# LPD-EPFL-ML/X-MAP

Hardware: AMD Instinct MI355X
Metric: item_sim_pairs_per_s (higher is better)
Workload: dtype f64

## Files before the change

### x-map_amd/csrc/tilesort.h

```cpp
#pragma once
#include "common.h"

namespace xmap {
namespace ts {

constexpr int BT = 256;
template <int RW> struct Chunk { static constexpr int CH = RW == 2 ? 4096 : 2048; static constexpr int EPT = CH / BT; };
constexpr int NB_LOG = 7;
constexpr int NB = 1 << NB_LOG;
constexpr int NA_MAX = 256;
constexpr int CAP = 3072;
constexpr int CT = 512;
constexpr int NK_MAX = 520;
constexpr int SL = 2048;
constexpr int LT = 256;

struct Geo {
    int K;
    long long M;
    int KW, ts_log, T, NA;
    int ch;
    const long long *ptr;
    int *tile_key0;
    long long *tile_pos0;
    int *tile_large;
    unsigned long long *curA;
    unsigned long long *curB;
    unsigned *counters;
    int2 *clist;
    int2 *slist;
    long long clist_cap, slist_cap;
};

__device__ __forceinline__ long long measure(const Geo &G, int k, long long p) { return p + (long long)k * G.KW; }

__device__ __forceinline__ void block_scan_2(const unsigned *cnt, unsigned *off, int n, unsigned *wsum) {
    const int tid = threadIdx.x, lane = tid & 63, w = tid >> 6;
    const unsigned a = (2 * tid < n) ? cnt[2 * tid] : 0u, b = (2 * tid + 1 < n) ? cnt[2 * tid + 1] : 0u;
    unsigned inc = a + b;
#pragma unroll
    for (int d = 1; d < 64; d <<= 1) { const unsigned o = __shfl_up(inc, d, 64); if (lane >= d) inc += o; }
    if (lane == 63) wsum[w] = inc;
    __syncthreads();
    unsigned base = 0;
    for (int x = 0; x < w; x++) base += wsum[x];
    const unsigned ex = base + inc - (a + b);
    if (2 * tid < n) off[2 * tid] = ex;
    if (2 * tid + 1 < n) off[2 * tid + 1] = ex + a;
    if (tid == BT - 1) off[n] = base + inc;
    __syncthreads();
}

template <int RW>
struct RecLoader {
    const unsigned long long *__restrict__ in;
    __device__ __forceinline__ bool chunk(long long n_in, long long &i0, long long &i1) const {
        i0 = (long long)blockIdx.x * Chunk<RW>::CH;
        i1 = min(n_in, i0 + Chunk<RW>::CH);
        return true;
    }
    __device__ __forceinline__ void load(long long idx, unsigned long long (&w)[RW]) const {
#pragma unroll
        for (int x = 0; x < RW; x++) w[x] = in[idx * RW + x];
    }
    __device__ __forceinline__ bool keep(const unsigned long long (&)[RW]) const { return true; }
    __device__ __forceinline__ void extra(long long, const unsigned long long (&)[Chunk<RW>::EPT][RW], const bool (&)[Chunk<RW>::EPT]) const {}
};

template <int RW, bool LEVEL_B, typename Loader>
__global__ __launch_bounds__(BT) void k_ts_bin(Geo G, Loader L, long long n_in, unsigned long long *__restrict__ out) {
    constexpr int CH = Chunk<RW>::CH, EPT = Chunk<RW>::EPT;
    constexpr int NBK = LEVEL_B ? 2 * NB : NA_MAX;
    __shared__ unsigned hist[NBK];
    __shared__ unsigned off[NBK + 1];
    __shared__ long long gbase[NBK];
    __shared__ unsigned wsum[BT / 64];
    __shared__ __attribute__((aligned(16))) unsigned long long stage[CH * RW];
    __shared__ unsigned short sbk[CH];
    constexpr int NKB = LEVEL_B ? NB : NA_MAX;
    __shared__ int bkey0[NKB], blarge[LEVEL_B ? NB : 1];
    const int tid = threadIdx.x;
    long long i0, i1;
    int a = 0;
    if (LEVEL_B) {
        if (blockIdx.x >= G.counters[0]) return;
        const int2 c = G.clist[blockIdx.x];
        a = c.x;
        const int t0 = a << NB_LOG, t1 = min(G.T, (a + 1) << NB_LOG);
        i0 = G.tile_pos0[t0] + (long long)c.y * CH;
        i1 = min(G.tile_pos0[t1], i0 + CH);
    } else {
        if (!L.chunk(n_in, i0, i1)) return;
    }
    const int nbk = LEVEL_B ? 2 * NB : G.NA;
    for (int b = tid; b < nbk; b += BT) hist[b] = 0u;
    if (LEVEL_B) {
        for (int b = tid; b < NB; b += BT) { bkey0[b] = G.tile_key0[(a << NB_LOG) + b]; blarge[b] = G.tile_large[(a << NB_LOG) + b]; }
    } else {
        for (int b = tid; b < NA_MAX; b += BT) bkey0[b] = b < G.NA ? G.tile_key0[b << NB_LOG] : 0x7fffffff;
    }
    __syncthreads();
    unsigned long long w[EPT][RW];
    bool on[EPT], rt[EPT];
    unsigned br[EPT];
#pragma unroll
    for (int r = 0; r < EPT; r++) {
        const long long idx = i0 + r * BT + tid;
        on[r] = idx < i1;
        if (on[r]) L.load(idx, w[r]);
        else {
#pragma unroll
            for (int x = 0; x < RW; x++) w[r][x] = 0ull;
        }
        rt[r] = on[r] && L.keep(w[r]);
    }
#pragma unroll
    for (int r = 0; r < EPT; r++) br[r] = 0u;
#pragma unroll
    for (int d = NKB / 2; d > 0; d >>= 1)
#pragma unroll
        for (int r = 0; r < EPT; r++)
            if (bkey0[br[r] + d] <= (int)(unsigned)w[r][0]) br[r] += d;
    if (LEVEL_B) {
#pragma unroll
        for (int r = 0; r < EPT; r++)
            if (blarge[br[r]] == (int)(unsigned)w[r][0]) br[r] |= NB;
    }
#pragma unroll
    for (int r = 0; r < EPT; r++)
        if (rt[r]) br[r] = (br[r] << 16) | atomicAdd(&hist[br[r]], 1u);
    __syncthreads();
    block_scan_2(hist, off, nbk, wsum);
    for (int b = tid; b < nbk; b += BT) {
        const unsigned c = hist[b];
        if (!c) continue;
        long long start;
        unsigned long long *cur;
        if (LEVEL_B) {
            const int t = (a << NB_LOG) | (b & (NB - 1));
            if (b >= NB) { start = G.ptr[G.tile_large[t]]; cur = &G.curB[(size_t)G.T + t]; }
            else { start = G.tile_pos0[t]; cur = &G.curB[t]; }
        } else {
            start = G.tile_pos0[b << NB_LOG];
            cur = &G.curA[b];
        }
        gbase[b] = (start + (long long)atomicAdd(cur, (unsigned long long)c) - (long long)off[b]) * RW;
    }
#pragma unroll
    for (int r = 0; r < EPT; r++) {
        if (!rt[r]) continue;
        const unsigned b = br[r] >> 16, s = off[b] + (br[r] & 0xffffu);
#pragma unroll
        for (int x = 0; x < RW; x++) stage[s * RW + x] = w[r][x];
        sbk[s] = (unsigned short)b;
    }
    L.extra(i0, w, on);
    __syncthreads();
    constexpr int VW = RW % 2 == 0 ? 2 : 1;
    const int nw = (int)off[nbk] * RW;
#pragma unroll 4
    for (int q = tid * VW; q < nw; q += BT * VW) {
        unsigned long long *o = out + (gbase[sbk[q / RW]] + q);
#pragma unroll
        for (int x = 0; x < VW; x++) o[x] = stage[q + x];
    }
}

struct TileHead { int k0, nk, large; long long pos0; int n; };
__device__ __forceinline__ TileHead tile_head(const Geo &G, int t) {
    TileHead h;
    h.k0 = G.tile_key0[t];
    const int k1 = G.tile_key0[t + 1];
    h.large = G.tile_large[t];
    const int ks1 = h.large >= 0 ? h.large : k1;
    h.nk = ks1 - h.k0;
    h.pos0 = G.tile_pos0[t];
    const long long pos1 = h.large >= 0 ? G.ptr[h.large] : G.tile_pos0[t + 1];
    h.n = (int)(pos1 - h.pos0);
    return h;
}

}
}
```

### x-map_amd/csrc/tri.h

```cpp
#pragma once
#include "common.h"
#include "tilesort.h"

namespace xmap {

constexpr int T_SLOTS = 1024;
constexpr int HMAX = 1024;
constexpr int SMALL_BOUND = 96;
constexpr int MID_BOUND = 384;

constexpr int N_CLASSES = 5;
constexpr int WIDE_MIN = 2048;
__host__ __device__ __forceinline__ int class_rank(int cls) {
    return cls == 4 ? 0 : (cls == 0 ? 1 : (cls == 2 ? 2 : (cls == 3 ? 3 : 4)));
}

__device__ __forceinline__ double weighted(double cs, int n, int cap) {
    const int mn = n < cap ? n : cap;
    return 1.0 * cs * (double)mn / (double)cap;
}
__device__ __forceinline__ unsigned long long ls_key(double d) {
    return (d != d) ? 0x7ff8000000000000ull : (unsigned long long)__double_as_longlong(d);
}

struct RaterRec { int e0; int pos_ge; float rating; int user; };
struct UbWide { int item_ge; int pad; double rating; };
struct RaterRecWide { int e0; int pos_ge; double rating; };

constexpr int COO_SHARDS = 4096;

int mirror_counts(hipStream_t st, int n_items, long long range_cap, int n_ranges, const unsigned long long *cur, const int *coo_i,
                  const int *coo_j, bool skip_self, int *part, int *counts, FillList *fills = nullptr);
void ts_geometry(int K, long long M, int ch, ts::Geo &G);
int ts_prepare(hipStream_t st, ts::Geo &G, const long long *ptr, FillList *fills = nullptr);
extern template __global__ void ts::k_ts_bin<3, true, ts::RecLoader<3>>(ts::Geo, ts::RecLoader<3>, long long, unsigned long long *__restrict__);

}
```

### x-map_amd/csrc/tri_layout.hip

```cpp
#include "tri.h"
#include "item_stats.h"

namespace xmap {

__device__ __forceinline__ unsigned long long wkey(int n, int item) {
    return ((unsigned long long)(unsigned)n << 32) | (unsigned)item;
}

constexpr int HIST_LDS = 2048;
constexpr int HIST_PER = 16;
__global__ __launch_bounds__(256) void k_hist(int I, const long long *iptr, int HB, int *hist) {
    __shared__ int loc[HIST_LDS];
    for (int t = threadIdx.x; t < HIST_LDS; t += 256) loc[t] = 0;
    __syncthreads();
    const long long base = (long long)blockIdx.x * 256 * HIST_PER;
    for (int q = 0; q < HIST_PER; q++) {
        const long long i = base + (long long)q * 256 + threadIdx.x;
        if (i < I) {
            long long n = iptr[i + 1] - iptr[i];
            int bin = n < HB - 1 ? (int)n : HB - 1;
            if (bin < HIST_LDS) atomicAdd(&loc[bin], 1); else atomicAdd(&hist[bin], 1);
        }
    }
    __syncthreads();
// ... 305 lines not shown
        int d = 0;
        if (u < U) { a = uptr[u]; d = (int)(uptr[u + 1] - a); }
        const bool small = d <= 16;
        int wmax = small ? d : 0;
#pragma unroll
        for (int m = 32; m >= 16; m >>= 1) wmax = max(wmax, __shfl_xor(wmax, m, 64));
        wmax = rl32(wmax, 0);
        if (wmax > 0) {
            unsigned long long key = 0ull;
            int px = 0;
            long long py = 0;
            if (small && gl < d) sort_entry3<WIDE>(uitem, ur32, ur64, cnt, a + gl, key, px, py);
            bitonic_desc3<WIDE>(pow2_at_least(wmax), gl, key, px, py);
            if (small && gl < d) emit_entry3<WIDE>(a, d, gl, u, px, py, ub, srec);
        }
    }
    for (int q = 0; q < 4; q++) {
        const long long u = u0 + q;
        if (u >= U) break;
        const long long a = uptr[u];
        const int d = (int)(uptr[u + 1] - a);
        if (d <= 16) continue;
        if (d <= 64) {
            unsigned long long key = 0ull;
            int px = 0;
            long long py = 0;
            if (lane < d) sort_entry3<WIDE>(uitem, ur32, ur64, cnt, a + lane, key, px, py);
            bitonic_desc3<WIDE>(pow2_at_least(d), lane, key, px, py);
            if (lane < d) emit_entry3<WIDE>(a, d, lane, u, px, py, ub, srec);
            continue;
        }
        unsigned long long *keys = d <= SORT_LDS ? lkeys[uniform((int)(threadIdx.x >> 6))] : ub_key + a;
        for (int p = lane; p < d; p += 64) {
            unsigned long long key;
            int px;
            long long py;
            sort_entry3<WIDE>(uitem, ur32, ur64, cnt, a + p, key, px, py);
            keys[p] = key;
        }
        __threadfence_block();
        for (int p = lane; p < d; p += 64) {
            unsigned long long key;
            int px;
            long long py;
            sort_entry3<WIDE>(uitem, ur32, ur64, cnt, a + p, key, px, py);
            int rank = 0;
            for (int o = 0; o < d; o++) rank += (keys[o] > key) || (keys[o] == key && o < p);
            emit_entry3<WIDE>(a, d, rank, u, px, py, ub, srec);
        }
    }
}

template <bool WIDE>
__device__ __forceinline__ ulonglong2 rater_record(const unsigned long long *w, const long long *uptr) {
    const unsigned user = WIDE ? (unsigned)w[2] : (unsigned)(w[1] >> 32);
    const unsigned e0 = (unsigned)uptr[user];
    ulonglong2 o;
    o.x = (unsigned long long)e0 | (w[0] & 0xffffffff00000000ull);
    o.y = w[1];
    return o;
}

template <bool WIDE>
__global__ __launch_bounds__(ts::CT) void k_rc_tiles(ts::Geo G, const unsigned long long *bufB, const long long *uptr,
                                                     ulonglong2 *rc, unsigned long long *Wp) {
    constexpr int RW = WIDE ? 3 : 2;
    __shared__ unsigned cur[ts::NK_MAX], kst[ts::NK_MAX];
    __shared__ unsigned long long wsum[ts::NK_MAX];
    __shared__ ulonglong2 lrec[ts::CAP];
    const ts::TileHead h = ts::tile_head(G, blockIdx.x);
    if (h.nk <= 0) return;
    for (int x = threadIdx.x; x < h.nk; x += ts::CT) {
        cur[x] = 0u; wsum[x] = 0ull;
        kst[x] = (unsigned)(G.ptr[h.k0 + x] - h.pos0);
    }
    __syncthreads();
    const bool in_lds = h.n <= ts::CAP;
    constexpr int UN = 4;
    for (int base = 0; base < h.n; base += ts::CT * UN) {
        unsigned long long w[UN][RW];
        bool on[UN];
#pragma unroll
        for (int t = 0; t < UN; t++) {
            const int idx = base + t * ts::CT + threadIdx.x;
            on[t] = idx < h.n;
            const size_t o = (size_t)(h.pos0 + (on[t] ? idx : 0)) * RW;
#pragma unroll
            for (int x = 0; x < RW; x++) w[t][x] = bufB[o + x];
        }
#pragma unroll
        for (int t = 0; t < UN; t++) {
            if (!on[t]) continue;
            const int kk = (int)((unsigned)w[t][0]) - h.k0;
            const unsigned q = kst[kk] + atomicAdd(&cur[kk], 1u);
            atomicAdd(&wsum[kk], (unsigned long long)((unsigned)(w[t][0] >> 32) & 0x7fffffffu));
            const ulonglong2 o = rater_record<WIDE>(w[t], uptr);
            if (in_lds) lrec[q] = o; else rc[h.pos0 + q] = o;
        }
    }
    __syncthreads();
    if (in_lds)
        for (int q = threadIdx.x; q < h.n; q += ts::CT) rc[h.pos0 + q] = lrec[q];
    for (int x = threadIdx.x; x < h.nk; x += ts::CT) Wp[h.k0 + x] = wsum[x];
}

template <bool WIDE>
__global__ __launch_bounds__(ts::LT) void k_rc_large(ts::Geo G, const unsigned long long *bufB, const long long *uptr,
                                                     ulonglong2 *rc, unsigned long long *Wp) {
    constexpr int RW = WIDE ? 3 : 2;
    if (blockIdx.x >= G.counters[1]) return;
    const int2 sl = G.slist[blockIdx.x];
    const long long lo = G.ptr[sl.x] + (long long)sl.y * ts::SL;
    const long long hi = min(G.ptr[sl.x + 1], lo + ts::SL);
    unsigned long long sum = 0ull;
    for (long long p = lo + threadIdx.x; p < hi; p += ts::LT) {
        unsigned long long w[RW];
#pragma unroll
        for (int x = 0; x < RW; x++) w[x] = bufB[(size_t)p * RW + x];
        sum += (unsigned long long)((unsigned)(w[0] >> 32) & 0x7fffffffu);
        rc[p] = rater_record<WIDE>(w, uptr);
    }
    sum = (unsigned long long)wave_sum_ll((long long)sum);
    if (lane_id() == 0 && sum) atomicAdd(&Wp[sl.x], sum);
}

struct RcSrc {
    RaterRec *rc; const double *u_avg;
    static constexpr bool has_flags = true;
    __device__ __forceinline__ void load(long long p, double &r, int &u) const { const RaterRec x = rc[p]; r = (double)x.rating; u = x.user; }
    __device__ __forceinline__ double uavg(int u) const { return u_avg[u]; }
    __device__ __forceinline__ void set_flag(long long p, bool ge) const { if (ge) rc[p].pos_ge |= (int)0x80000000u; }
};
struct RcWideSrc {
    const RaterRecWide *rc;
    static constexpr bool has_flags = false;
    __device__ __forceinline__ void load(long long p, double &r, int &u) const { r = rc[p].rating; u = 0; }
    __device__ __forceinline__ double uavg(int) const { return 0.0; }
    __device__ __forceinline__ void set_flag(long long, bool) const {}
};

constexpr int STAT_BIG = 512;
constexpr int STAT_CHK = 2048;
struct BigList {
    unsigned *counters;
    int2 *chunks;
    int4 *items;
    double *part;
    long long chunk_cap, item_cap;
};

template <typename Src>
__global__ __launch_bounds__(256) void k_item_stats3(int I, int lo, int hi, const long long *iptr, const Src src, double *info,
                                                     double *norms, BigList B) {
    const int i0 = lo + (blockIdx.x * 4 + uniform((int)(threadIdx.x >> 6))) * 4;
    if (i0 >= hi) return;
    const int lane = lane_id();
    {
        const int i = i0 + (lane >> 4);
        const bool on = i < hi && iptr[i + 1] - iptr[i] <= 64;
        item_stats_group<16, Src, false>(on, i, lane & 15, I, iptr, src, info, norms, nullptr, nullptr);
    }
    for (int t = 0; t < 4; t++) {
        const int i = i0 + t;
        if (i >= hi) break;
        const long long n = iptr[i + 1] - iptr[i];
        if (n <= 64) continue;
        if (n > STAT_BIG) {
            if (lane == 0) {
                const int nch = (int)((n + STAT_CHK - 1) / STAT_CHK);
                const unsigned base = atomicAdd(&B.counters[0], (unsigned)nch);
                const unsigned slot = atomicAdd(&B.counters[1], 1u);
                if ((long long)slot < B.item_cap) B.items[slot] = make_int4(i, (int)base, nch, 0);
                for (int x = 0; x < nch; x++)
                    if ((long long)base + x < B.chunk_cap) B.chunks[base + x] = make_int2(i, x);
            }
            continue;
        }
// ... 112 lines not shown
        FillList F;
        heavy_set_fills(F, n_users, hist, ctl);
        int rc = fill_multi(st, F);
        if (rc) return rc;
    }
    if (I > 0) {
        k_hist<<<dim3((unsigned)((I + 256 * HIST_PER - 1) / (256 * HIST_PER))), dim3(256), 0, st>>>(I, (const long long *)item_ptr, HB, hist);
        XM_LAUNCH_CHECK();
    }
    int rcode = xmap_exclusive_scan_i32_to_i64(stream, hist, pre, HB, nullptr);
    if (rcode) return rcode;
    if (HB - 1 > ch_min) {
        k_threshold<<<dim3((unsigned)((HB + 255) / 256)), dim3(256), 0, st>>>(I, HB, (const long long *)pre, ch_min, ctl);
        XM_LAUNCH_CHECK();
    }
    if (I > 0) {
        k_mark_heavy<<<dim3((unsigned)((I + 255) / 256)), dim3(256), 0, st>>>(I, (const long long *)item_ptr, ctl, hid, hlist, ctl + 1);
        XM_LAUNCH_CHECK();
    }
    return XMAP_OK;
}

int read_heavy_ctl(hipStream_t st, const int32_t *ctl, int32_t *h_ctl) {
    XM_HIP(hipMemcpyAsync(h_ctl, ctl, 2 * sizeof(int32_t), hipMemcpyDeviceToHost, st));
    XM_HIP(hipStreamSynchronize(st));
    if (h_ctl[1] > HMAX) {
        set_error("heavy set larger than %d", HMAX);
        return XMAP_ERR_OVERFLOW;
    }
    return XMAP_OK;
}

int plan_rows(void *stream, const xmap_ratings *R, int32_t slot_target, const void *rc, const int64_t *pre, const int32_t *hid,
              const int32_t *ctl, int32_t *Q, int32_t *C, uint8_t *small, uint64_t *Wp, int32_t *Qcat, int64_t *uq_ptr, int64_t *uc_ptr,
              int32_t dups, int64_t *h_light, int64_t *h_heavy) {
    XM_ARG(slot_target > 0 && slot_target <= T_SLOTS);
    hipStream_t st = (hipStream_t)stream;
    const int I = R->n_items;
    if (I > 0) {
        k_plan2<<<dim3((unsigned)((I + 255) / 256)), dim3(256), 0, st>>>(
            I, (const long long *)R->item_ptr, (const RaterRec *)rc, (const long long *)pre, (int)R->n_users + 2, hid, ctl, slot_target, dups,
            Q, C, small, (unsigned long long *)Wp, Qcat);
        XM_LAUNCH_CHECK();
    }
    int rcode = xmap_exclusive_scan_i32_to_i64(stream, Qcat, uq_ptr, (int64_t)N_CLASSES * I, h_light);
    if (rcode) return rcode;
    return xmap_exclusive_scan_i32_to_i64(stream, C, uc_ptr, I, h_heavy);
}

template <int RW>
int sort_rater_records(hipStream_t st, const ts::Geo &G, long long nnz, const void *srec, void *bufA, void *bufB, const int64_t *user_ptr,
                       void *rc, uint64_t *Wp) {
    constexpr bool WIDE = RW == 3;
    const dim3 gridA((unsigned)((nnz + G.ch - 1) / G.ch)), gridB((unsigned)G.clist_cap), gridL((unsigned)G.slist_cap);
    ts::RecLoader<RW> LA{(const unsigned long long *)srec}, LB{(const unsigned long long *)bufA};
    ts::k_ts_bin<RW, false, ts::RecLoader<RW>><<<gridA, dim3(ts::BT), 0, st>>>(G, LA, nnz, (unsigned long long *)bufA);
    XM_LAUNCH_CHECK();
    ts::k_ts_bin<RW, true, ts::RecLoader<RW>><<<gridB, dim3(ts::BT), 0, st>>>(G, LB, nnz, (unsigned long long *)bufB);
    XM_LAUNCH_CHECK();
    k_rc_tiles<WIDE><<<dim3((unsigned)G.T), dim3(ts::CT), 0, st>>>(G, (const unsigned long long *)bufB, (const long long *)user_ptr,
                                                                  (ulonglong2 *)rc, (unsigned long long *)Wp);
    XM_LAUNCH_CHECK();
    k_rc_large<WIDE><<<gridL, dim3(ts::LT), 0, st>>>(G, (const unsigned long long *)bufB, (const long long *)user_ptr, (ulonglong2 *)rc,
                                                     (unsigned long long *)Wp);
    XM_LAUNCH_CHECK();
    return XMAP_OK;
}

template <typename Src>
int item_stats3(hipStream_t st, int I, int lo, int hi, const int64_t *item_ptr, const Src &src, double *info, double *norms,
                const BigList &B) {
    const long long *iptr = (const long long *)item_ptr;
    const dim3 grid((unsigned)((hi - lo + 15) / 16)), gridC((unsigned)((B.chunk_cap + 3) / 4)), gridI((unsigned)((B.item_cap + 63) / 64));
    k_item_stats3<Src><<<grid, dim3(256), 0, st>>>(I, lo, hi, iptr, src, info, norms, B);
    XM_LAUNCH_CHECK();
    k_item_chunks<Src><<<gridC, dim3(256), 0, st>>>(iptr, src, B);
    XM_LAUNCH_CHECK();
    k_item_big<<<gridI, dim3(64), 0, st>>>(I, B, info, norms);
    XM_LAUNCH_CHECK();
    if constexpr (Src::has_flags) {
        k_item_big_flags<Src><<<gridC, dim3(256), 0, st>>>(iptr, src, B, info);
        XM_LAUNCH_CHECK();
    }
    return XMAP_OK;
}

}

extern "C" {

int xmap_sim2_layout(void *stream, const xmap_ratings *R, const double *info, int32_t ch_min, int32_t *hist ,
                     int64_t *pre , int32_t *ctl , int32_t *hid, int32_t *hlist ,
                     uint64_t *ub_key , void *ub , void *rc ,
                     uint64_t *Wp , int32_t dups, int32_t *h_ctl ) {
    XM_ARG(R && info && hist && pre && ctl && hid && hlist && ub_key && ub && rc && Wp && ch_min >= 64);
    XM_ARG(R->nnz < 0x7fffffffLL && R->n_users < 0x7ffffff0LL);
    hipStream_t st = (hipStream_t)stream;
    const int I = R->n_items;
    int rcode = heavy_set(stream, I, R->n_users, R->item_ptr, ch_min, hist, pre, ctl, hid, hlist);
    if (rcode) return rcode;
    if (R->n_users > 0) {
        k_sort_profiles<<<dim3((unsigned)((R->n_users + 15) / 16)), dim3(256), 0, st>>>(
            R->n_users, (const long long *)R->user_ptr, R->user_item, R->user_rating, (const long long *)R->item_ptr, info,
            (unsigned long long *)ub_key, (int2 *)ub);
        XM_LAUNCH_CHECK();
    }
    XM_HIP(hipMemsetAsync(Wp, 0, sizeof(uint64_t) * (size_t)(I > 0 ? I : 1), st));
    if (R->nnz > 0) {
        if (dups) XM_HIP(hipMemsetAsync(ub_key, 0, sizeof(int32_t) * (size_t)R->nnz, st));
        k_rater_records<<<dim3((unsigned)((R->nnz + 255) / 256)), dim3(256), 0, st>>>(
            I, R->nnz, (const long long *)R->item_ptr, R->item_user, (const long long *)R->user_ptr, (const int2 *)ub,
            (RaterRec *)rc, dups ? (int *)ub_key : nullptr, (unsigned long long *)Wp);
        XM_LAUNCH_CHECK();
    }
    return h_ctl ? read_heavy_ctl(st, ctl, h_ctl) : XMAP_OK;
}

// ... 172 lines not shown
```

### x-map_amd/csrc/tri_mirror.hip

```cpp
#include "tri.h"

namespace xmap {

constexpr int SC_U = 4;
__global__ __launch_bounds__(256) void k_scatter(long long n, const int *coo_i, const int *coo_j, const double *coo_sim,
                                                 const int *coo_mutu, const int *coo_nij, const double *coo_aux,
                                                 const long long *row_ptr, int *fill, int *col, double *sim, int *mutu,
                                                 int *nij, double *aux) {
    const int lane = lane_id();
    const long long r0 = ((long long)blockIdx.x * (blockDim.x >> 6) + uniform((int)(threadIdx.x >> 6))) * (64 * SC_U) + lane;
    int i[SC_U], j[SC_U], m[SC_U], nn[SC_U];
    double s[SC_U], x[SC_U];
    bool valid[SC_U];
#pragma unroll
    for (int u = 0; u < SC_U; u++) {
        const long long r = r0 + 64 * u;
        i[u] = (r < n) ? coo_i[r] : -1;
    }
#pragma unroll
    for (int u = 0; u < SC_U; u++) {
        const long long r = r0 + 64 * u;
        valid[u] = i[u] >= 0;
        j[u] = 0; m[u] = 0; nn[u] = 0; s[u] = 0.0; x[u] = 0.0;
        if (valid[u]) {
// ... 273 lines not shown
    __shared__ double laux[AUX ? CAPX : 1];
    __shared__ int lcol[CAPX], lmutu[CAPX], lnij[CAPX];
    __shared__ unsigned short lkk[CAPX];
    const ts::TileHead h = ts::tile_head(G, blockIdx.x);
    if (h.nk <= 0 || h.n <= 0) return;
    for (int x = threadIdx.x; x < h.nk; x += ts::CT) {
        const int k = h.k0 + x;
        cur[x] = 0u;
        kst[x] = (unsigned)(G.ptr[k] - h.pos0);
        gsh[x] = row_ptr[k] + own[k] - G.ptr[k];
    }
    __syncthreads();
    const bool in_lds = h.n <= CAPX;
    constexpr int UN = 4;
    for (int base = 0; base < h.n; base += ts::CT * UN) {
        unsigned long long w[UN][RW];
        bool on[UN];
#pragma unroll
        for (int t = 0; t < UN; t++) {
            const int idx = base + t * ts::CT + threadIdx.x;
            on[t] = idx < h.n;
            const size_t o = (size_t)(h.pos0 + (on[t] ? idx : 0)) * RW;
#pragma unroll
            for (int x = 0; x < RW; x++) w[t][x] = bufB[o + x];
        }
#pragma unroll
        for (int t = 0; t < UN; t++) {
            if (!on[t]) continue;
            const int kk = (int)((unsigned)w[t][0]) - h.k0;
            const unsigned q = kst[kk] + atomicAdd(&cur[kk], 1u);
            const int ci = (int)(w[t][0] >> 32), cm = (int)(unsigned)w[t][2], cn = (int)(w[t][2] >> 32);
            const double cs = __longlong_as_double((long long)w[t][1]);
            const double ca = AUX ? __longlong_as_double((long long)w[t][RW - 1]) : 0.0;
            if (in_lds) {
                lcol[q] = ci; lsim[q] = cs; lmutu[q] = cm; lnij[q] = cn; lkk[q] = (unsigned short)kk;
                if (AUX) laux[q] = ca;
            } else {
                const long long P = h.pos0 + q + gsh[kk];
                col[P] = ci; sim[P] = cs; mutu[P] = cm; nij[P] = cn;
                if (AUX) aux[P] = ca;
            }
        }
    }
    if (!in_lds) return;
    __syncthreads();
    for (int q = threadIdx.x; q < h.n; q += ts::CT) {
        const long long P = h.pos0 + q + gsh[lkk[q]];
        col[P] = lcol[q]; sim[P] = lsim[q]; mutu[P] = lmutu[q]; nij[P] = lnij[q];
        if (AUX) aux[P] = laux[q];
    }
}

template <bool AUX>
__global__ __launch_bounds__(ts::LT) void k_mir_large(ts::Geo G, const unsigned long long *bufB, const long long *row_ptr,
                                                      const int *own, int *col, double *sim, int *mutu, int *nij, double *aux) {
    constexpr int RW = AUX ? 4 : 3;
    if (blockIdx.x >= G.counters[1]) return;
    const int2 sl = G.slist[blockIdx.x];
    const int k = sl.x;
    const long long lo = G.ptr[k] + (long long)sl.y * ts::SL;
    const long long hi = min(G.ptr[k + 1], lo + ts::SL);
    const long long sh = row_ptr[k] + own[k] - G.ptr[k];
    for (long long p = lo + threadIdx.x; p < hi; p += ts::LT) {
        const unsigned long long w0 = bufB[(size_t)p * RW], w1 = bufB[(size_t)p * RW + 1], w2 = bufB[(size_t)p * RW + 2];
        const long long P = p + sh;
        col[P] = (int)(w0 >> 32); sim[P] = __longlong_as_double((long long)w1);
        mutu[P] = (int)(unsigned)w2; nij[P] = (int)(w2 >> 32);
        if (AUX) aux[P] = __longlong_as_double((long long)bufB[(size_t)p * RW + 3]);
    }
}

namespace ts {

__global__ __launch_bounds__(256) void k_ts_plan(Geo G) {
    const int k = blockIdx.x * blockDim.x + threadIdx.x;
    if (k >= G.K) return;
    const long long p = G.ptr[k], cnt = G.ptr[k + 1] - p;
    const int t = (int)(measure(G, k, p) >> G.ts_log);
    const bool large = cnt >= (1ll << G.ts_log);
    const int tp = k > 0 ? (int)(measure(G, k - 1, G.ptr[k - 1]) >> G.ts_log) : -1;
    for (int x = tp + 1; x <= t; x++) { G.tile_key0[x] = k; G.tile_pos0[x] = p; }
    if (k == G.K - 1)
        for (int x = t + 1; x <= G.T; x++) { G.tile_key0[x] = G.K; G.tile_pos0[x] = G.ptr[G.K]; }
    if (large) {
        G.tile_large[t] = k;
        const int nsl = (int)((cnt + SL - 1) / SL);
        const unsigned base = atomicAdd(&G.counters[1], (unsigned)nsl);
        for (int x = 0; x < nsl; x++)
            if ((long long)base + x < G.slist_cap) G.slist[base + x] = make_int2(k, x);
    }
}

__global__ __launch_bounds__(256) void k_ts_chunks(Geo G) {
    const int a = blockIdx.x * blockDim.x + threadIdx.x;
    if (a >= G.NA) return;
    const int t0 = a << NB_LOG, t1 = min(G.T, (a + 1) << NB_LOG);
    const long long size = G.tile_pos0[t1] - G.tile_pos0[t0];
    const int nch = (int)((size + G.ch - 1) / G.ch);
    if (nch == 0) return;
    const unsigned base = atomicAdd(&G.counters[0], (unsigned)nch);
    for (int x = 0; x < nch; x++)
        if ((long long)base + x < G.clist_cap) G.clist[base + x] = make_int2(a, x);
}

}

template __global__ void ts::k_ts_bin<3, true, ts::RecLoader<3>>(ts::Geo, ts::RecLoader<3>, long long, unsigned long long *__restrict__);

void ts_geometry(int K, long long M, int ch, ts::Geo &G) {
    G.K = K; G.M = M; G.ch = ch;
    G.ts_log = 11;
    for (;;) {
        const long long TS = 1ll << G.ts_log;
        long long kw = M / (4 * (long long)(K > 0 ? K : 1));
        const long long kw_min = TS / (ts::NK_MAX - 2) + 1;
        if (kw < kw_min) kw = kw_min;
        if (kw < 4) kw = 4;
        const long long tiles = ((M + (long long)K * kw) >> G.ts_log) + 1;
        if (tiles <= (long long)ts::NA_MAX * ts::NB || G.ts_log >= 30) {
            G.KW = (int)kw;
            G.NA = (int)((tiles + ts::NB - 1) / ts::NB);
            if (G.NA < 1) G.NA = 1;
            if (G.NA > ts::NA_MAX) G.NA = ts::NA_MAX;
            G.T = G.NA * ts::NB;
            return;
        }
        G.ts_log++;
    }
}

int ts_prepare(hipStream_t st, ts::Geo &G, const long long *ptr, FillList *fills) {
    G.ptr = ptr;
    G.clist_cap = G.M / G.ch + G.NA + 1;
    G.slist_cap = G.M / ts::SL + (G.M >> G.ts_log) + 2;
    XM_HIP(xm_malloc_async((void **)&G.tile_key0, sizeof(int) * ((size_t)G.T + 1), st));
    XM_HIP(xm_malloc_async((void **)&G.tile_pos0, sizeof(long long) * ((size_t)G.T + 1), st));
    XM_HIP(xm_malloc_async((void **)&G.tile_large, sizeof(int) * (size_t)G.T, st));
    unsigned long long *z = nullptr;
    const size_t nz = (size_t)G.NA + 2 * (size_t)G.T + 1;
    XM_HIP(xm_malloc_async((void **)&z, sizeof(unsigned long long) * nz, st));
    G.curA = z; G.curB = z + G.NA; G.counters = (unsigned *)(z + G.NA + 2 * (size_t)G.T);
    XM_HIP(xm_malloc_async((void **)&G.clist, sizeof(int2) * (size_t)G.clist_cap, st));
    XM_HIP(xm_malloc_async((void **)&G.slist, sizeof(int2) * (size_t)G.slist_cap, st));
    FillList own;
    FillList &F = fills ? *fills : own;
    F.add(z, sizeof(unsigned long long) * nz);
    F.add(G.tile_large, sizeof(int) * (size_t)G.T, 0xffffffffu);
    int rcode = fill_multi(st, F);
    if (rcode) return rcode;
    ts::k_ts_plan<<<dim3((unsigned)((G.K + 255) / 256)), dim3(256), 0, st>>>(G);
    XM_LAUNCH_CHECK();
    ts::k_ts_chunks<<<dim3((unsigned)((G.NA + 255) / 256)), dim3(256), 0, st>>>(G);
    XM_LAUNCH_CHECK();
    return XMAP_OK;
}

namespace {
template <bool AUX, bool SHARE>
int mirror_levels(hipStream_t st, const ts::Geo &G, int64_t coo_cap, const int32_t *coo_i, const int32_t *coo_j, const double *coo_sim,
                  const int32_t *coo_mutu, const int32_t *coo_nij, const double *coo_aux, const longlong2 *chunks, const unsigned *n_chunks,
                  long long chunk_cap, int64_t n_pairs, const int32_t *own, const int64_t *row_ptr, int32_t *fill, void *bufA, void *bufB,
                  int32_t *col, double *sim, int32_t *mutu, int32_t *nij, double *aux, int row_lo, int row_hi) {
    constexpr int RW = AUX ? 4 : 3;
    CooLoaderT<AUX, SHARE> LA{coo_i, coo_j, coo_sim, coo_mutu, coo_nij, coo_aux, chunks, n_chunks, (const long long *)row_ptr, fill,
                              col, sim, mutu, nij, aux, row_lo, row_hi};
    ts::RecLoader<RW> LB{(const unsigned long long *)bufA};
    ts::k_ts_bin<RW, false, CooLoaderT<AUX, SHARE>><<<dim3((unsigned)chunk_cap), dim3(ts::BT), 0, st>>>(G, LA, coo_cap, (unsigned long long *)bufA);
    XM_LAUNCH_CHECK();
    ts::k_ts_bin<RW, true, ts::RecLoader<RW>><<<dim3((unsigned)G.clist_cap), dim3(ts::BT), 0, st>>>(G, LB, n_pairs, (unsigned long long *)bufB);
    XM_LAUNCH_CHECK();
    k_mir_tiles<AUX><<<dim3((unsigned)G.T), dim3(ts::CT), 0, st>>>(G, (const unsigned long long *)bufB, (const long long *)row_ptr, own, col,
                                                                   sim, mutu, nij, aux);
    XM_LAUNCH_CHECK();
    k_mir_large<AUX><<<dim3((unsigned)G.slist_cap), dim3(ts::LT), 0, st>>>(G, (const unsigned long long *)bufB, (const long long *)row_ptr, own,
                                                                            col, sim, mutu, nij, aux);
    XM_LAUNCH_CHECK();
    return XMAP_OK;
}
}

int mirror_counts(hipStream_t st, int n_items, long long range_cap, int n_ranges, const unsigned long long *cur, const int *coo_i,
                  const int *coo_j, bool skip_self, int *part, int *counts, FillList *fills) {
    FillList own;
    FillList &F = fills ? *fills : own;
    if (n_items <= 0 || range_cap <= 0 || n_ranges <= 0) return fill_multi(st, F);
    int sh = 0;
    while (((long long)(n_items - 1) >> sh) >= CB_MAX) sh++;
    unsigned *bcnt = nullptr, *bcur = nullptr;
    long long *bptr = nullptr;
    XM_HIP(xm_malloc_async((void **)&bcnt, sizeof(unsigned) * CB_MAX, st));
    XM_HIP(xm_malloc_async((void **)&bcur, sizeof(unsigned) * CB_MAX, st));
    XM_HIP(xm_malloc_async((void **)&bptr, sizeof(long long) * (CB_MAX + 1), st));
    F.add(bcnt, sizeof(unsigned) * CB_MAX);
    int rcode = fill_multi(st, F);
    if (rcode) return rcode;
    const long long segs = (long long)n_ranges * ((range_cap + CB_CHUNK - 1) / CB_CHUNK);
    const dim3 g((unsigned)((segs + CB_SPB - 1) / CB_SPB));
    (skip_self ? k_cbs_hist<true> : k_cbs_hist<false>)<<<g, dim3(CB_T), 0, st>>>(range_cap, n_ranges, cur, coo_i, coo_j, sh, bcnt);
    XM_LAUNCH_CHECK();
    k_cb_scan<<<dim3(1), dim3(CB_MAX), 0, st>>>(bcnt, bptr, bcur);
    XM_LAUNCH_CHECK();
    (skip_self ? k_cbs_scatter<true> : k_cbs_scatter<false>)<<<g, dim3(CB_T), 0, st>>>(range_cap, n_ranges, cur, coo_i, coo_j, sh, bptr, bcur,
                                                                                        part);
    XM_LAUNCH_CHECK();
    const long long cap = range_cap * n_ranges;
    k_cb_count<<<dim3((unsigned)((cap + (long long)CB_CHUNK * CB_SPB - 1) / ((long long)CB_CHUNK * CB_SPB))), dim3(CB_T), 0, st>>>(
        -1, part, sh, bptr, n_items, counts);
    XM_LAUNCH_CHECK();
    return XMAP_OK;
}

}

using namespace xmap;

extern "C" {

int xmap_sim2_scatter(void *stream, int32_t n_items, int64_t n_coo, const int32_t *coo_i, const int32_t *coo_j,
                      const double *coo_sim, const int32_t *coo_mutu, const int32_t *coo_nij, const double *coo_ls ,
                      const int64_t *row_ptr, int32_t *fill , const int32_t *hid, const int32_t *hlist,
                      int32_t *col, double *sim, int32_t *mutu, int32_t *nij, double *ls ) {
    XM_ARG(coo_i && coo_j && coo_sim && coo_mutu && coo_nij && row_ptr && fill && hid && hlist && col && sim && mutu && nij);
    XM_ARG((coo_ls != nullptr) == (ls != nullptr));
    hipStream_t st = (hipStream_t)stream;
    XM_HIP(hipMemsetAsync(fill, 0, sizeof(int32_t) * (size_t)(n_items > 0 ? n_items : 1), st));
    if (n_coo > 0) {
        k_scatter<<<dim3((unsigned)((n_coo + 256 * SC_U - 1) / (256 * SC_U))), dim3(256), 0, st>>>(
            n_coo, coo_i, coo_j, coo_sim, coo_mutu, coo_nij, coo_ls, (const long long *)row_ptr, fill, col, sim, mutu, nij, ls);
// ... 61 lines not shown
```

### x-map_amd/csrc/util.hip

```cpp
#include <stdarg.h>
#include <stdlib.h>
#include <vector>

#include "common.h"

namespace xmap {
static thread_local char g_err[512] = "";
void set_error(const char *fmt, ...) {
    va_list ap;
    va_start(ap, fmt);
    vsnprintf(g_err, sizeof(g_err), fmt, ap);
    va_end(ap);
}

namespace {
struct Chunk { char *base; size_t size, used; };
struct Arena { int dev; hipStream_t st; std::vector<Chunk> chunks; size_t live; };
thread_local std::vector<Arena> g_arenas;
constexpr size_t ARENA_KEEP = (size_t)256 << 20;
Arena *arena_find(int dev, hipStream_t st) {
    for (Arena &a : g_arenas) if (a.dev == dev && a.st == st) return &a;
    return nullptr;
}
Arena *arena_of(hipStream_t st) {
// ... 214 lines not shown
        v[k] = (base + k < n) ? S.load(y, base + k) : 0;
        s += v[k];
    }
    long long tot;
    long long ex = block_exclusive_scan(s, &tot, smem) + off;
#pragma unroll
    for (int k = 0; k < SCAN_ITEMS; k++) {
        if (base + k < n) out[base + k] = ex;
        ex += v[k];
    }
    if (SELF && blockIdx.x == gridDim.x - 1 && threadIdx.x == 0) out[n] = off + tot;
}

template <typename TIn>
static int exclusive_scan(hipStream_t st, int n_arrays, const TIn *in0, const TIn *in1, int plus, int64_t *out0, int64_t *out1, int64_t n,
                          int64_t *h_total) {
    XM_ARG(n >= 0 && (n_arrays == 1 || n_arrays == 2));
    XM_SCOPE(st);
    const int64_t n_tiles = (n + SCAN_TILE - 1) / SCAN_TILE;
    XM_ARG(n_tiles < 0x7fffffffLL);
    const ScanIn<TIn> S{in0, in1, plus};
    if (n_tiles == 0) {
        XM_HIP(hipMemsetAsync(out0 + n, 0, sizeof(int64_t), st));
        if (n_arrays == 2) XM_HIP(hipMemsetAsync(out1 + n, 0, sizeof(int64_t), st));
    } else {
        long long *tile = nullptr;
        XM_HIP(xm_malloc_async((void **)&tile, sizeof(long long) * (size_t)n_tiles * (size_t)n_arrays, st));
        const dim3 grid((unsigned)n_tiles, (unsigned)n_arrays);
        k_tile_sums<TIn><<<grid, dim3(SCAN_THREADS), 0, st>>>(S, n, n_tiles, tile);
        XM_LAUNCH_CHECK();
        if (n_tiles <= SCAN2_MAX_TILES) {
            k_tile_scan<TIn, true><<<grid, dim3(SCAN_THREADS), 0, st>>>(S, n, n_tiles, tile, (long long *)out0, (long long *)out1);
            XM_LAUNCH_CHECK();
        } else {
            k_scan_tile_sums<<<dim3(1, (unsigned)n_arrays), dim3(SCAN_THREADS), 0, st>>>(tile, n_tiles, (long long *)(out0 + n),
                                                                                          (long long *)(out1 ? out1 + n : nullptr));
            XM_LAUNCH_CHECK();
            k_tile_scan<TIn, false><<<grid, dim3(SCAN_THREADS), 0, st>>>(S, n, n_tiles, tile, (long long *)out0, (long long *)out1);
            XM_LAUNCH_CHECK();
        }
        XM_HIP(xm_free_async(tile, st));
    }
    if (h_total) {
        XM_HIP(hipMemcpyAsync(h_total, out0 + n, sizeof(int64_t), hipMemcpyDeviceToHost, st));
        if (n_arrays == 2) XM_HIP(hipMemcpyAsync(h_total + 1, out1 + n, sizeof(int64_t), hipMemcpyDeviceToHost, st));
        XM_HIP(hipStreamSynchronize(st));
    }
    return XMAP_OK;
}
}

extern "C" {
const char *xmap_last_error(void) { return xmap::g_err; }
int xmap_version(void) { return 114; }

int xmap_trim(void) {
    XM_HIP(hipDeviceSynchronize());
    int dev = 0;
    XM_HIP(hipGetDevice(&dev));
    for (xmap::Arena &a : xmap::g_arenas) {
        if (a.dev != dev || a.live != 0) continue;
        for (xmap::Chunk &c : a.chunks) (void)hipFree(c.base);
        a.chunks.clear();
    }
    return XMAP_OK;
}

int xmap_debug_arena(void *stream, int64_t *live, int64_t *reserved) {
    XM_ARG(live && reserved);
    int dev = 0;
    XM_HIP(hipGetDevice(&dev));
    *live = 0; *reserved = 0;
    if (xmap::Arena *a = xmap::arena_find(dev, (hipStream_t)stream)) {
        *live = (int64_t)a->live;
        for (xmap::Chunk &c : a->chunks) *reserved += (int64_t)c.size;
    }
    return XMAP_OK;
}
int xmap_debug_arena_call(void *stream, int64_t bytes, int fail) {
    using namespace xmap;
    XM_SCOPE(stream);
    hipStream_t st = (hipStream_t)stream;
    void *a = nullptr, *b = nullptr;
    XM_HIP(xm_malloc_async(&a, (size_t)bytes, st));
    XM_HIP(xm_malloc_async(&b, 1024, st));
    XM_ARG(!fail);
    XM_HIP(xm_free_async(b, st));
    XM_HIP(xm_free_async(a, st));
    return XMAP_OK;
}

int xmap_exclusive_scan_i64(void *stream, const int64_t *in, int64_t *out, int64_t n, int64_t *h_total) {
    XM_ARG(out && (in || n == 0));
    return xmap::exclusive_scan<long long>((hipStream_t)stream, 1, (const long long *)in, nullptr, 0, out, nullptr, n, h_total);
}
int xmap_exclusive_scan_i32_to_i64(void *stream, const int32_t *in, int64_t *out, int64_t n, int64_t *h_total) {
    XM_ARG(out && (in || n == 0));
    return xmap::exclusive_scan<int>((hipStream_t)stream, 1, in, nullptr, 0, out, nullptr, n, h_total);
}
int xmap_exclusive_scan2_i32_to_i64(void *stream, const int32_t *in_a, const int32_t *in_b, int32_t a_plus_b, int64_t *out_a,
                                    int64_t *out_b, int64_t n, int64_t *h_totals) {
    XM_ARG(out_a && out_b && ((in_a && in_b) || n == 0));
    return xmap::exclusive_scan<int>((hipStream_t)stream, 2, in_a, in_b, a_plus_b ? 1 : 0, out_a, out_b, n, h_totals);
}
int xmap_scan_self_tiles(void) { return xmap::SCAN2_MAX_TILES; }
}
```

Measured before the change: 26.22 billion.

## Fuse large-key finalization into level-B tile-sort binning kernel

```diff
diff --git a/x-map_amd/csrc/tilesort.h b/x-map_amd/csrc/tilesort.h
--- a/x-map_amd/csrc/tilesort.h
+++ b/x-map_amd/csrc/tilesort.h
@@ -12,8 +12,6 @@
 constexpr int CAP = 3072;
 constexpr int CT = 512;
 constexpr int NK_MAX = 520;
-constexpr int SL = 2048;
-constexpr int LT = 256;
 
 struct Geo {
     int K;
@@ -28,8 +26,7 @@
     unsigned long long *curB;
     unsigned *counters;
     int2 *clist;
-    int2 *slist;
-    long long clist_cap, slist_cap;
+    long long clist_cap;
 };
 
 __device__ __forceinline__ long long measure(const Geo &G, int k, long long p) { return p + (long long)k * G.KW; }
@@ -67,8 +64,17 @@
     __device__ __forceinline__ void extra(long long, const unsigned long long (&)[Chunk<RW>::EPT][RW], const bool (&)[Chunk<RW>::EPT]) const {}
 };
 
-template <int RW, bool LEVEL_B, typename Loader>
-__global__ __launch_bounds__(BT) void k_ts_bin(Geo G, Loader L, long long n_in, unsigned long long *__restrict__ out) {
+struct NoFin {
+    static constexpr bool STATE = false, WSUM = false;
+    __device__ __forceinline__ long long state(const Geo &, int) const { return 0; }
+    template <int RW> __device__ __forceinline__ unsigned gather(const unsigned long long (&)[RW]) const { return 0u; }
+    template <int RW> __device__ __forceinline__ unsigned long long store(long long, long long, const unsigned long long (&)[RW], unsigned) const { return 0ull; }
+    __device__ __forceinline__ void flush(int, unsigned long long) const {}
+};
+constexpr int FU = 4;
+
+template <int RW, bool LEVEL_B, typename Loader, typename Fin>
+__global__ __launch_bounds__(BT) void k_ts_bin(Geo G, Loader L, long long n_in, unsigned long long *__restrict__ out, Fin F) {
     constexpr int CH = Chunk<RW>::CH, EPT = Chunk<RW>::EPT;
     constexpr int NBK = LEVEL_B ? 2 * NB : NA_MAX;
     __shared__ unsigned hist[NBK];
@@ -79,6 +85,8 @@
     __shared__ unsigned short sbk[CH];
     constexpr int NKB = LEVEL_B ? NB : NA_MAX;
     __shared__ int bkey0[NKB], blarge[LEVEL_B ? NB : 1];
+    __shared__ long long fstate[LEVEL_B && Fin::STATE ? NB : 1];
+    __shared__ unsigned long long fsum[LEVEL_B && Fin::WSUM ? NB : 1];
     const int tid = threadIdx.x;
     long long i0, i1;
     int a = 0;
@@ -94,6 +102,8 @@
     }
     const int nbk = LEVEL_B ? 2 * NB : G.NA;
     for (int b = tid; b < nbk; b += BT) hist[b] = 0u;
+    if (LEVEL_B && Fin::WSUM)
+        for (int b = tid; b < NB; b += BT) fsum[b] = 0ull;
     if (LEVEL_B) {
         for (int b = tid; b < NB; b += BT) { bkey0[b] = G.tile_key0[(a << NB_LOG) + b]; blarge[b] = G.tile_large[(a << NB_LOG) + b]; }
     } else {
@@ -144,7 +154,13 @@
             start = G.tile_pos0[b << NB_LOG];
             cur = &G.curA[b];
         }
-        gbase[b] = (start + (long long)atomicAdd(cur, (unsigned long long)c) - (long long)off[b]) * RW;
+        const long long pos = start + (long long)atomicAdd(cur, (unsigned long long)c) - (long long)off[b];
+        if (LEVEL_B && b >= NB) {
+            gbase[b] = pos;
+            if (Fin::STATE) fstate[b - NB] = F.state(G, blarge[b - NB]);
+        } else {
+            gbase[b] = pos * RW;
+        }
     }
 #pragma unroll
     for (int r = 0; r < EPT; r++) {
@@ -157,12 +173,49 @@
     L.extra(i0, w, on);
     __syncthreads();
     constexpr int VW = RW % 2 == 0 ? 2 : 1;
-    const int nw = (int)off[nbk] * RW;
+    const int nw = (int)off[LEVEL_B ? NB : nbk] * RW;
 #pragma unroll 4
     for (int q = tid * VW; q < nw; q += BT * VW) {
         unsigned long long *o = out + (gbase[sbk[q / RW]] + q);
 #pragma unroll
         for (int x = 0; x < VW; x++) o[x] = stage[q + x];
+    }
+    if (!LEVEL_B) return;
+    const int s0 = (int)off[NB], s1 = (int)off[2 * NB];
+    for (int sw = s0 + (tid & ~63); sw < s1; sw += BT * FU) {
+        const int sb = sw + (tid & 63);
+        unsigned long long v[FU][RW];
+        unsigned g[FU];
+        int bk[FU];
+#pragma unroll
+        for (int t = 0; t < FU; t++) {
+            const int s = min(sb + t * BT, s1 - 1);
+            bk[t] = sbk[s];
+#pragma unroll
+            for (int x = 0; x < RW; x++) v[t][x] = stage[s * RW + x];
+        }
+#pragma unroll
+        for (int t = 0; t < FU; t++) g[t] = F.gather(v[t]);
+#pragma unroll
+        for (int t = 0; t < FU; t++) {
+            if (sw + t * BT >= s1) break;
+            const int s = sb + t * BT;
+            unsigned long long add = 0ull;
+            if (s < s1) add = F.store(Fin::STATE ? fstate[bk[t] - NB] : 0ll, gbase[bk[t]] + s, v[t], g[t]);
+            if (Fin::WSUM) {
+                if (__all(bk[t] == __builtin_amdgcn_readfirstlane(bk[t]))) {
+                    add = (unsigned long long)wave_sum_ll((long long)add);
+                    if (lane_id() == 0 && add) atomicAdd(&fsum[bk[t] - NB], add);
+                } else if (add) {
+                    atomicAdd(&fsum[bk[t] - NB], add);
+                }
+            }
+        }
+    }
+    if (Fin::WSUM && s1 > s0) {
+        __syncthreads();
+        for (int b = tid; b < NB; b += BT)
+            if (hist[NB + b]) F.flush(blarge[b], fsum[b]);
     }
 }
 
diff --git a/x-map_amd/csrc/tri.h b/x-map_amd/csrc/tri.h
--- a/x-map_amd/csrc/tri.h
+++ b/x-map_amd/csrc/tri.h
@@ -33,6 +33,5 @@
                   const int *coo_j, bool skip_self, int *part, int *counts, FillList *fills = nullptr);
 void ts_geometry(int K, long long M, int ch, ts::Geo &G);
 int ts_prepare(hipStream_t st, ts::Geo &G, const long long *ptr, FillList *fills = nullptr);
-extern template __global__ void ts::k_ts_bin<3, true, ts::RecLoader<3>>(ts::Geo, ts::RecLoader<3>, long long, unsigned long long *__restrict__);
 
 }
diff --git a/x-map_amd/csrc/tri_layout.hip b/x-map_amd/csrc/tri_layout.hip
--- a/x-map_amd/csrc/tri_layout.hip
+++ b/x-map_amd/csrc/tri_layout.hip
@@ -381,13 +381,17 @@
 }
 
 template <bool WIDE>
-__device__ __forceinline__ ulonglong2 rater_record(const unsigned long long *w, const long long *uptr) {
-    const unsigned user = WIDE ? (unsigned)w[2] : (unsigned)(w[1] >> 32);
-    const unsigned e0 = (unsigned)uptr[user];
+__device__ __forceinline__ unsigned rater_user(const unsigned long long *w) { return WIDE ? (unsigned)w[2] : (unsigned)(w[1] >> 32); }
+template <bool WIDE>
+__device__ __forceinline__ ulonglong2 rater_record_at(const unsigned long long *w, unsigned e0) {
     ulonglong2 o;
     o.x = (unsigned long long)e0 | (w[0] & 0xffffffff00000000ull);
     o.y = w[1];
     return o;
+}
+template <bool WIDE>
+__device__ __forceinline__ ulonglong2 rater_record(const unsigned long long *w, const long long *uptr) {
+    return rater_record_at<WIDE>(w, (unsigned)uptr[rater_user<WIDE>(w)]);
 }
 
 template <bool WIDE>
@@ -434,24 +438,18 @@
 }
 
 template <bool WIDE>
-__global__ __launch_bounds__(ts::LT) void k_rc_large(ts::Geo G, const unsigned long long *bufB, const long long *uptr,
-                                                     ulonglong2 *rc, unsigned long long *Wp) {
-    constexpr int RW = WIDE ? 3 : 2;
-    if (blockIdx.x >= G.counters[1]) return;
-    const int2 sl = G.slist[blockIdx.x];
-    const long long lo = G.ptr[sl.x] + (long long)sl.y * ts::SL;
-    const long long hi = min(G.ptr[sl.x + 1], lo + ts::SL);
-    unsigned long long sum = 0ull;
-    for (long long p = lo + threadIdx.x; p < hi; p += ts::LT) {
-        unsigned long long w[RW];
-#pragma unroll
-        for (int x = 0; x < RW; x++) w[x] = bufB[(size_t)p * RW + x];
-        sum += (unsigned long long)((unsigned)(w[0] >> 32) & 0x7fffffffu);
-        rc[p] = rater_record<WIDE>(w, uptr);
-    }
-    sum = (unsigned long long)wave_sum_ll((long long)sum);
-    if (lane_id() == 0 && sum) atomicAdd(&Wp[sl.x], sum);
-}
+struct RcFin {
+    static constexpr int RW = WIDE ? 3 : 2;
+    static constexpr bool STATE = false, WSUM = true;
+    const long long *__restrict__ uptr; ulonglong2 *__restrict__ rc; unsigned long long *Wp;
+    __device__ __forceinline__ long long state(const ts::Geo &, int) const { return 0; }
+    __device__ __forceinline__ unsigned gather(const unsigned long long (&w)[RW]) const { return (unsigned)uptr[rater_user<WIDE>(w)]; }
+    __device__ __forceinline__ unsigned long long store(long long, long long p, const unsigned long long (&w)[RW], unsigned e0) const {
+        rc[p] = rater_record_at<WIDE>(w, e0);
+        return (unsigned long long)((unsigned)(w[0] >> 32) & 0x7fffffffu);
+    }
+    __device__ __forceinline__ void flush(int k, unsigned long long sum) const { if (sum) atomicAdd(&Wp[k], sum); }
+};
 
 struct RcSrc {
     RaterRec *rc; const double *u_avg;
@@ -670,17 +668,15 @@
 int sort_rater_records(hipStream_t st, const ts::Geo &G, long long nnz, const void *srec, void *bufA, void *bufB, const int64_t *user_ptr,
                        void *rc, uint64_t *Wp) {
     constexpr bool WIDE = RW == 3;
-    const dim3 gridA((unsigned)((nnz + G.ch - 1) / G.ch)), gridB((unsigned)G.clist_cap), gridL((unsigned)G.slist_cap);
+    const dim3 gridA((unsigned)((nnz + G.ch - 1) / G.ch)), gridB((unsigned)G.clist_cap);
     ts::RecLoader<RW> LA{(const unsigned long long *)srec}, LB{(const unsigned long long *)bufA};
-    ts::k_ts_bin<RW, false, ts::RecLoader<RW>><<<gridA, dim3(ts::BT), 0, st>>>(G, LA, nnz, (unsigned long long *)bufA);
+    RcFin<WIDE> FB{(const long long *)user_ptr, (ulonglong2 *)rc, (unsigned long long *)Wp};
+    ts::k_ts_bin<RW, false, ts::RecLoader<RW>, ts::NoFin><<<gridA, dim3(ts::BT), 0, st>>>(G, LA, nnz, (unsigned long long *)bufA, ts::NoFin{});
     XM_LAUNCH_CHECK();
-    ts::k_ts_bin<RW, true, ts::RecLoader<RW>><<<gridB, dim3(ts::BT), 0, st>>>(G, LB, nnz, (unsigned long long *)bufB);
+    ts::k_ts_bin<RW, true, ts::RecLoader<RW>, RcFin<WIDE>><<<gridB, dim3(ts::BT), 0, st>>>(G, LB, nnz, (unsigned long long *)bufB, FB);
     XM_LAUNCH_CHECK();
     k_rc_tiles<WIDE><<<dim3((unsigned)G.T), dim3(ts::CT), 0, st>>>(G, (const unsigned long long *)bufB, (const long long *)user_ptr,
                                                                   (ulonglong2 *)rc, (unsigned long long *)Wp);
-    XM_LAUNCH_CHECK();
-    k_rc_large<WIDE><<<gridL, dim3(ts::LT), 0, st>>>(G, (const unsigned long long *)bufB, (const long long *)user_ptr, (ulonglong2 *)rc,
-                                                     (unsigned long long *)Wp);
     XM_LAUNCH_CHECK();
     return XMAP_OK;
 }
diff --git a/x-map_amd/csrc/tri_mirror.hip b/x-map_amd/csrc/tri_mirror.hip
--- a/x-map_amd/csrc/tri_mirror.hip
+++ b/x-map_amd/csrc/tri_mirror.hip
@@ -349,23 +349,22 @@
 }
 
 template <bool AUX>
-__global__ __launch_bounds__(ts::LT) void k_mir_large(ts::Geo G, const unsigned long long *bufB, const long long *row_ptr,
-                                                      const int *own, int *col, double *sim, int *mutu, int *nij, double *aux) {
-    constexpr int RW = AUX ? 4 : 3;
-    if (blockIdx.x >= G.counters[1]) return;
-    const int2 sl = G.slist[blockIdx.x];
-    const int k = sl.x;
-    const long long lo = G.ptr[k] + (long long)sl.y * ts::SL;
-    const long long hi = min(G.ptr[k + 1], lo + ts::SL);
-    const long long sh = row_ptr[k] + own[k] - G.ptr[k];
-    for (long long p = lo + threadIdx.x; p < hi; p += ts::LT) {
-        const unsigned long long w0 = bufB[(size_t)p * RW], w1 = bufB[(size_t)p * RW + 1], w2 = bufB[(size_t)p * RW + 2];
+struct MirFin {
+    static constexpr int RW = AUX ? 4 : 3;
+    static constexpr bool STATE = true, WSUM = false;
+    const long long *__restrict__ row_ptr; const int *__restrict__ own;
+    int *__restrict__ col; double *__restrict__ sim; int *__restrict__ mutu; int *__restrict__ nij; double *__restrict__ aux;
+    __device__ __forceinline__ long long state(const ts::Geo &G, int k) const { return row_ptr[k] + (long long)own[k] - G.ptr[k]; }
+    __device__ __forceinline__ unsigned gather(const unsigned long long (&)[RW]) const { return 0u; }
+    __device__ __forceinline__ unsigned long long store(long long sh, long long p, const unsigned long long (&w)[RW], unsigned) const {
         const long long P = p + sh;
-        col[P] = (int)(w0 >> 32); sim[P] = __longlong_as_double((long long)w1);
-        mutu[P] = (int)(unsigned)w2; nij[P] = (int)(w2 >> 32);
-        if (AUX) aux[P] = __longlong_as_double((long long)bufB[(size_t)p * RW + 3]);
-    }
-}
+        col[P] = (int)(w[0] >> 32); sim[P] = __longlong_as_double((long long)w[1]);
+        mutu[P] = (int)(unsigned)w[2]; nij[P] = (int)(w[2] >> 32);
+        if (AUX) aux[P] = __longlong_as_double((long long)w[RW - 1]);
+        return 0ull;
+    }
+    __device__ __forceinline__ void flush(int, unsigned long long) const {}
+};
 
 namespace ts {
 
@@ -379,13 +378,7 @@
     for (int x = tp + 1; x <= t; x++) { G.tile_key0[x] = k; G.tile_pos0[x] = p; }
     if (k == G.K - 1)
         for (int x = t + 1; x <= G.T; x++) { G.tile_key0[x] = G.K; G.tile_pos0[x] = G.ptr[G.K]; }
-    if (large) {
-        G.tile_large[t] = k;
-        const int nsl = (int)((cnt + SL - 1) / SL);
-        const unsigned base = atomicAdd(&G.counters[1], (unsigned)nsl);
-        for (int x = 0; x < nsl; x++)
-            if ((long long)base + x < G.slist_cap) G.slist[base + x] = make_int2(k, x);
-    }
+    if (large) G.tile_large[t] = k;
 }
 
 __global__ __launch_bounds__(256) void k_ts_chunks(Geo G) {
@@ -401,8 +394,6 @@
 }
 
 }
-
-template __global__ void ts::k_ts_bin<3, true, ts::RecLoader<3>>(ts::Geo, ts::RecLoader<3>, long long, unsigned long long *__restrict__);
 
 void ts_geometry(int K, long long M, int ch, ts::Geo &G) {
     G.K = K; G.M = M; G.ch = ch;
@@ -429,7 +420,6 @@
 int ts_prepare(hipStream_t st, ts::Geo &G, const long long *ptr, FillList *fills) {
     G.ptr = ptr;
     G.clist_cap = G.M / G.ch + G.NA + 1;
-    G.slist_cap = G.M / ts::SL + (G.M >> G.ts_log) + 2;
     XM_HIP(xm_malloc_async((void **)&G.tile_key0, sizeof(int) * ((size_t)G.T + 1), st));
     XM_HIP(xm_malloc_async((void **)&G.tile_pos0, sizeof(long long) * ((size_t)G.T + 1), st));
     XM_HIP(xm_malloc_async((void **)&G.tile_large, sizeof(int) * (size_t)G.T, st));
@@ -438,7 +428,6 @@
     XM_HIP(xm_malloc_async((void **)&z, sizeof(unsigned long long) * nz, st));
     G.curA = z; G.curB = z + G.NA; G.counters = (unsigned *)(z + G.NA + 2 * (size_t)G.T);
     XM_HIP(xm_malloc_async((void **)&G.clist, sizeof(int2) * (size_t)G.clist_cap, st));
-    XM_HIP(xm_malloc_async((void **)&G.slist, sizeof(int2) * (size_t)G.slist_cap, st));
     FillList own;
     FillList &F = fills ? *fills : own;
     F.add(z, sizeof(unsigned long long) * nz);
@@ -462,15 +451,15 @@
     CooLoaderT<AUX, SHARE> LA{coo_i, coo_j, coo_sim, coo_mutu, coo_nij, coo_aux, chunks, n_chunks, (const long long *)row_ptr, fill,
                               col, sim, mutu, nij, aux, row_lo, row_hi};
     ts::RecLoader<RW> LB{(const unsigned long long *)bufA};
-    ts::k_ts_bin<RW, false, CooLoaderT<AUX, SHARE>><<<dim3((unsigned)chunk_cap), dim3(ts::BT), 0, st>>>(G, LA, coo_cap, (unsigned long long *)bufA);
-    XM_LAUNCH_CHECK();
-    ts::k_ts_bin<RW, true, ts::RecLoader<RW>><<<dim3((unsigned)G.clist_cap), dim3(ts::BT), 0, st>>>(G, LB, n_pairs, (unsigned long long *)bufB);
+    MirFin<AUX> FB{(const long long *)row_ptr, own, col, sim, mutu, nij, aux};
+    ts::k_ts_bin<RW, false, CooLoaderT<AUX, SHARE>, ts::NoFin><<<dim3((unsigned)chunk_cap), dim3(ts::BT), 0, st>>>(
+        G, LA, coo_cap, (unsigned long long *)bufA, ts::NoFin{});
+    XM_LAUNCH_CHECK();
+    ts::k_ts_bin<RW, true, ts::RecLoader<RW>, MirFin<AUX>><<<dim3((unsigned)G.clist_cap), dim3(ts::BT), 0, st>>>(
+        G, LB, n_pairs, (unsigned long long *)bufB, FB);
     XM_LAUNCH_CHECK();
     k_mir_tiles<AUX><<<dim3((unsigned)G.T), dim3(ts::CT), 0, st>>>(G, (const unsigned long long *)bufB, (const long long *)row_ptr, own, col,
                                                                    sim, mutu, nij, aux);
-    XM_LAUNCH_CHECK();
-    k_mir_large<AUX><<<dim3((unsigned)G.slist_cap), dim3(ts::LT), 0, st>>>(G, (const unsigned long long *)bufB, (const long long *)row_ptr, own,
-                                                                            col, sim, mutu, nij, aux);
     XM_LAUNCH_CHECK();
     return XMAP_OK;
 }
diff --git a/x-map_amd/csrc/util.hip b/x-map_amd/csrc/util.hip
--- a/x-map_amd/csrc/util.hip
+++ b/x-map_amd/csrc/util.hip
@@ -290,7 +290,7 @@
 
 extern "C" {
 const char *xmap_last_error(void) { return xmap::g_err; }
-int xmap_version(void) { return 114; }
+int xmap_version(void) { return 115; }
 
 int xmap_trim(void) {
     XM_HIP(hipDeviceSynchronize());
```

Result: faster. 27.44 billion, median of 6 (+4.7%).
